# 0xastro/Cognitive-Radio-Network

Hardware: AMD Instinct MI355X
Metric: Msamples/s IQ through FFT+energy-detect, 4096-pt x 3ch; % HBM roofline (higher is better)
Workload: dtype f32

## Files before the change

### cognitive-radio-network_amd/csrc/crn_api.cpp

```cpp
#include <algorithm>
#include <cmath>
#include <cstdio>
#include <cstring>
#include <string>
#include <vector>

#include "crn_forms.h"
#include "crn_handle.h"
#include "crn_segments.h"

namespace crn {
static thread_local std::string g_err;
int fail(int code, const std::string &msg) {
  g_err = msg;
  return code;
}
}

void crn::handle_geometry(crn_handle *h, int *fft_len, int *device) {
  std::lock_guard<std::mutex> lk(h->tables_mu);
  *fft_len = h->cfg.fft_len;
  *device = h->device;
}

// ... 122 lines not shown
    h->tail_groups_per_wg = variant - 300;
    return CRN_OK;
  }
  if (variant >= 400 && variant <= 402) {
    h->deal_max_epochs = variant == 400 ? -1 : variant == 401 ? 0 : (int64_t)0x7fffffff;
    return CRN_OK;
  }
  if (variant < 0 || variant > crn::sense_num_variants()) return crn::fail(CRN_ERR_ARG, "variant out of range");
  if (!crn::sense_variant_available(variant))
    return crn::fail(CRN_ERR_ARG, "variant " + std::to_string(variant) + " is not a form of this library: the measurement variants (7, 17, 19-22, 26, 27) "
                                  "are compiled into libcrnsense_ab.so (make -C csrc ab), not into the shipped library; any other number names "
                                  "a form that no longer exists");
  h->variant = variant;
  return CRN_OK;
}

static void fill_plan_facts(const crn_handle *h, bool spectrum, crn::SenseParams &p) {
  p.hann_sym = h->cfg.window == CRN_WINDOW_HANN;
  p.aligned_shift = spectrum ? 0 : h->aligned_shift;
  p.acc_mask = h->variant == 2 ? 0xFFFFu : h->acc_mask;
  p.n_row_entries = h->n_row_entries;
  p.n_row_entries_shift = h->n_row_entries_shift;
  p.acc_mask_shift = h->variant == 2 ? 0xFFFFu : h->acc_mask_shift;
  p.cfar_on = h->cfar_on ? 1 : 0;
}

int crn_sense_kernel_info(crn_handle *h, char *name, int32_t name_len, int32_t *threads_per_block,
                          int32_t *lds_bytes, int32_t *epochs_per_block) {
  if (!h) return crn::fail(CRN_ERR_ARG, "null handle");
  std::lock_guard<std::mutex> lk(h->tables_mu);
  crn::SenseParams p{};
  p.L = h->cfg.fft_len;
  fill_plan_facts(h, false, p);
  const std::optional<crn::FormKey> k = crn::select_form(
      crn::make_form_query(p, h->cfg.fft_len, h->cfg.mode == CRN_MODE_REF_MAG, h->cfg.window != CRN_WINDOW_RECT, h->variant, false));
  if (!k) return crn::fail(CRN_ERR_STATE, "no kernel form for this handle");
  const crn::FormGeometry g = crn::form_geometry(*k);
  if (threads_per_block) *threads_per_block = g.threads;
  if (lds_bytes) *lds_bytes = g.lds_bytes;
  if (epochs_per_block) *epochs_per_block = g.epochs_per_block;
  if (name && name_len > 0) crn::form_name(*k, name, (size_t)name_len);
  return CRN_OK;
}

static int resolve_strides(const crn_handle *h, int32_t L, int64_t *epoch_stride, int *frame_stride) {
  const crn_cfg &c = h->cfg;
// ... 400 lines not shown
```

### cognitive-radio-network_amd/csrc/crn_butterflies.h

```cpp
#ifndef CRN_BUTTERFLIES_H
#define CRN_BUTTERFLIES_H
#include <hip/hip_runtime.h>
#include <type_traits>
#include <stdint.h>

#include "crn_forms.h"

namespace crn {

typedef float cx __attribute__((ext_vector_type(2)));
#define CRN_DEV static __device__ __forceinline__
#define CRN_HD static __host__ __device__ __forceinline__

#define CRN_C1 0.92387953251128674f
#define CRN_S1 0.38268343236508977f
#define CRN_H_ 0.70710678118654752f

#define CRN_PK_ADD "v_pk_add_f32 %0, %1, %2"
#define CRN_PK_SUB "v_pk_add_f32 %0, %1, %2 neg_lo:[0,1] neg_hi:[0,1]"
#define CRN_PK_ADD_MJ "v_pk_add_f32 %0, %1, %2 op_sel:[0,1] op_sel_hi:[1,0] neg_hi:[0,1]"
#define CRN_PK_SUB_MJ "v_pk_add_f32 %0, %1, %2 op_sel:[0,1] op_sel_hi:[1,0] neg_lo:[0,1]"
#define CRN_PK_MUL_T "v_pk_mul_f32 %0, %1, %2 op_sel_hi:[1,0]"
#define CRN_PK_MUL_D "v_pk_fma_f32 %0, %1, %2, %3 op_sel:[1,1,0] op_sel_hi:[0,1,1] neg_lo:[1,0,0]"
#define CRN_PK_MULCONJ_D "v_pk_fma_f32 %0, %1, %2, %3 op_sel:[1,1,0] op_sel_hi:[0,1,1] neg_hi:[1,0,0]"
// ... 157 lines not shown
CRN_HD void dft16_hann(const cx (&in)[16], cx (&out)[16], const cx (&wp)[4], const Hook &hook = Hook()) {
  using m = M<PK>;
  cx y[16];
#pragma unroll
  for (int i = 0; i < 16; i++) y[i] = in[i];
  static_for<4>([&](auto rc) {
    constexpr int r0 = decltype(rc)::value;
    constexpr int S = r0 & 1;
    const cx x0 = y[r0], x1 = y[r0 + 4], x2 = y[r0 + 8], x3 = y[r0 + 12];
    const cx w0 = wp[r0 / 2], w1 = wp[(r0 + 4) / 2];
    const cx s02 = m::template fma_w<S, false>(w0, m::sub(x0, x2), x2);
    const cx d02 = m::template fma_w<S, true>(w0, m::add(x0, x2), x2);
    const cx s13 = m::template fma_w<S, false>(w1, m::sub(x1, x3), x3);
    const cx d13 = m::template fma_w<S, true>(w1, m::add(x1, x3), x3);
    y[r0] = m::add(s02, s13);
    y[r0 + 8] = m::sub(s02, s13);
    y[r0 + 4] = m::add_mj(d02, d13);
    y[r0 + 12] = m::sub_mj(d02, d13);
    hook(r0);
  });
  dft16_level_b<PK>(y, out, hook);
}

template <bool PK, unsigned MASK>
CRN_HD void dft16_pruned(const cx (&in)[16], cx (&out)[16]) {
  using m = M<PK>;
  cx y[16];
#pragma unroll
  for (int i = 0; i < 16; i++) y[i] = in[i];
#pragma unroll
  for (int r0 = 0; r0 < 4; r0++) dft4<PK>(y[r0], y[r0 + 4], y[r0 + 8], y[r0 + 12]);
  const cx w1 = {CRN_C1, -CRN_S1}, w3 = {CRN_S1, -CRN_C1}, w9 = {-CRN_C1, CRN_S1};
  static_for<4>([&](auto ac) {
    constexpr int a0 = decltype(ac)::value;
    constexpr bool n0 = (MASK >> (a0 + 0)) & 1, n1 = (MASK >> (a0 + 4)) & 1, n2 = (MASK >> (a0 + 8)) & 1, n3 = (MASK >> (a0 + 12)) & 1;
    constexpr bool S = n0 || n2, D = n1 || n3;
    const cx b0 = y[4 * a0];
    if constexpr (a0 == 2) {
      const cx p = m::add_mj(y[9], y[9]), q = m::sub_mj(y[11], y[11]);
      if constexpr (S) {
        const cx s02 = m::add_mj(b0, y[10]), u = m::sub(p, q);
        if constexpr (n0) out[a0 + 0] = m::fma_h(u, s02);
        if constexpr (n2) out[a0 + 8] = m::fms_h(u, s02);
      }
      if constexpr (D) {
        const cx d02 = m::sub_mj(b0, y[10]), v = m::add(p, q);
        if constexpr (n1) out[a0 + 4] = m::fma_h_mj(v, d02);
        if constexpr (n3) out[a0 + 12] = m::fms_h_mj(v, d02);
      }
    } else {
      cx b1 = y[4 * a0 + 1], b3 = y[4 * a0 + 3];
      if constexpr (a0 == 1) { b1 = m::mul_c(b1, w1); b3 = m::mul_c(b3, w3); }
      if constexpr (a0 == 3) { b1 = m::mul_c(b1, w3); b3 = m::mul_c(b3, w9); }
      const cx r = a0 == 1 ? m::add_mj(y[4 * a0 + 2], y[4 * a0 + 2]) : a0 == 3 ? m::sub_mj(y[4 * a0 + 2], y[4 * a0 + 2]) : y[4 * a0 + 2];
      if constexpr (S) {
        const cx s02 = a0 == 0 ? m::add(b0, r) : a0 == 1 ? m::fma_h(r, b0) : m::fms_h(r, b0);
        const cx s13 = m::add(b1, b3);
        if constexpr (n0) out[a0 + 0] = m::add(s02, s13);
        if constexpr (n2) out[a0 + 8] = m::sub(s02, s13);
      }
      if constexpr (D) {
        const cx d02 = a0 == 0 ? m::sub(b0, r) : a0 == 1 ? m::fms_h(r, b0) : m::fma_h(r, b0);
        const cx d13 = m::sub(b1, b3);
        if constexpr (n1) out[a0 + 4] = m::add_mj(d02, d13);
        if constexpr (n3) out[a0 + 12] = m::sub_mj(d02, d13);
      }
    }
  });
}

template <bool PK, unsigned MSK, bool B2MJ = false>
CRN_HD void dft4_pruned(cx &a0, cx &a1, cx &a2, cx &a3) {
  using m = M<PK>;
  constexpr bool S = (MSK & 5u) != 0, D = (MSK & 10u) != 0;
  cx s02 = a0, d02 = a0, s13 = a1, d13 = a1;
  if constexpr (S) { s02 = B2MJ ? m::add_mj(a0, a2) : m::add(a0, a2); s13 = m::add(a1, a3); }
  if constexpr (D) { d02 = B2MJ ? m::sub_mj(a0, a2) : m::sub(a0, a2); d13 = m::sub(a1, a3); }
  if constexpr ((MSK & 1u) != 0) a0 = m::add(s02, s13);
  if constexpr ((MSK & 4u) != 0) a2 = m::sub(s02, s13);
  if constexpr ((MSK & 2u) != 0) a1 = m::add_mj(d02, d13);
  if constexpr ((MSK & 8u) != 0) a3 = m::sub_mj(d02, d13);
}

template <bool PK, unsigned M8>
CRN_HD void dft8_pruned(const cx (&in)[8], cx (&out)[8]) {
  using m = M<PK>;
  cx y[8];
#pragma unroll
  for (int i = 0; i < 8; i++) y[i] = in[i];
  constexpr unsigned need = (M8 | (M8 >> 4)) & 15u;
  dft4_pruned<PK, need>(y[0], y[2], y[4], y[6]);
  dft4_pruned<PK, need>(y[1], y[3], y[5], y[7]);
  if constexpr ((M8 & 0x01u) != 0) out[0] = m::add(y[0], y[1]);
  if constexpr ((M8 & 0x10u) != 0) out[4] = m::sub(y[0], y[1]);
  if constexpr ((M8 & 0x22u) != 0) {
    const cx p = m::add_mj(y[3], y[3]);
    if constexpr ((M8 & 0x02u) != 0) out[1] = m::fma_h(p, y[2]);
    if constexpr ((M8 & 0x20u) != 0) out[5] = m::fms_h(p, y[2]);
  }
  if constexpr ((M8 & 0x04u) != 0) out[2] = m::add_mj(y[4], y[5]);
  if constexpr ((M8 & 0x40u) != 0) out[6] = m::sub_mj(y[4], y[5]);
  if constexpr ((M8 & 0x88u) != 0) {
    const cx q = m::sub_mj(y[7], y[7]);
    if constexpr ((M8 & 0x08u) != 0) out[3] = m::fms_h(q, y[6]);
    if constexpr ((M8 & 0x80u) != 0) out[7] = m::fma_h(q, y[6]);
  }
// ... 24 lines not shown
```

### cognitive-radio-network_amd/csrc/crn_epoch_close.h

```cpp
#ifndef CRN_EPOCH_CLOSE_H
#define CRN_EPOCH_CLOSE_H
#include "crn_frame.h"

#ifdef CRN_AB_VARIANTS
#include "crn_frame_ab.h"
#else
namespace crn {
template <class C>
struct CloseTrace {
  CRN_DEV void workgroup_start(const SenseParams &, int) {}
  CRN_DEV void enter(const SenseParams &, long long, bool, int, int) {}
  CRN_DEV void stamp1() {}
  CRN_DEV void stamp2() {}
  CRN_DEV void stamp3() {}
  CRN_DEV void leave(const SenseParams &, long long, bool, int) {}
};
}
#endif

namespace crn {

template <int R3>
struct CloseImage {
  static constexpr int kFeat = spec_phys(Geo<R3>::N);
// ... 189 lines not shown
    constexpr auto next_live = [](int d) {
      for (int x = d + 1; x < R3; x++)
        for (int j = 0; j < J; j++)
          if ((acc_mask<C>() >> (j * R3 + x)) & 1u) return x;
      return (int)R3;
    };
    constexpr int kFirst = next_live(-1);
    float fsum = 0.f;
    constexpr bool SHIFTED = BinMap<C>::S != 0;
    constexpr int kEnt0 = SHIFTED ? 0 : kTabRowEntries;
    const int *ent_tab = SHIFTED ? p.row_entries_shift : p.band_tab;
    typename SWords<CAP>::T ent_next = s_load_row<CAP, (kEnt0 + kFirst * CAP) * 4>(ent_tab);
    static_for<R3>([&](auto dc) {
      constexpr int d = decltype(dc)::value;
      if constexpr (row_live(d)) {
        typename SWords<CAP>::T ent = ent_next;
        s_wait_row(ent);
        constexpr int dn = next_live(d);
        if constexpr (dn < R3) ent_next = s_load_row<CAP, (kEnt0 + dn * CAP) * 4>(ent_tab);
#pragma unroll
        for (int e = 0; e < CAP; e++) {
          const int w = ent[e];
          if (w != 0) {
            const int band = w >> 18, lo = (w >> 9) & 511, span = (w & 511) - lo;
            float v = 0.f;
#pragma unroll
            for (int j = 0; j < J; j++) {
              if (((AM >> (j * R3 + d)) & 1u) == 0) continue;
              const int base = BinMap<C>::q(a, m_lo, j);
              v += (unsigned)(base - lo) < (unsigned)span ? acc[j * R3 + d] : 0.f;
            }
            v = team_sum<TEAM>(v, tid);
            fsum += lane == band ? v : 0.f;
          }
        }
      }
    });
#pragma unroll
    for (int i = 0; i < 16; i++) acc[i] = 0.f;
    trace.stamp1();
    if constexpr (TPG > 1) {
      if (lane < 16) part[(tid / TEAM) * 16 + lane] = fsum;
      __syncthreads();
      trace.stamp2();
      if (t < TEAM && lane < 16) {
        thr_lane = thr[lane];
        fsum = 0.f;
#pragma unroll
        for (int w = 0; w < TPG; w++) fsum += part[(grp * TPG + w) * 16 + lane];
      }
    }
    trace.stamp3();
// ... 344 lines not shown
```

### cognitive-radio-network_amd/csrc/crn_forms.h

```cpp
#ifndef CRN_FORMS_H
#define CRN_FORMS_H
#include <optional>

#include "crn_kernels.h"

namespace crn {

enum : int {
  kSpread = 4,
  kLdsBlk = 32,
  kTw1C = 64,
  kRows = 256,
  kMulti = 512,
  kPrioValu = 1024,
#ifdef CRN_AB_VARIANTS
  kTrace = 4096,
#endif
  kRegBands = 8192,
  kHannSym = 16384,
  kTw2Early = 32768,
  kAlignedBands = 65536,
  kSc16 = 131072,
  kDeal = 1048576,
  kCfar = 2097152,
};

static constexpr unsigned kRefPlanRows = 0x8267u;

constexpr unsigned ref_acc_mask_shifted(int R3, int S) {
  const int seg[5][2] = {{0, 16}, {496, 511}, {55, 85}, {189, 222}, {300, 310}};
  const int J = 16 / R3, Sc = R3 / 2, N = 256 * R3;
  unsigned mask = 0;
  for (int s = 0; s < 5; s++)
    for (int k = seg[s][0] * Sc; k < seg[s][1] * Sc; k++) {
      const int ks = (k + S) & (N - 1);
      mask |= 1u << ((((ks & 255) >> 4) % J) * R3 + (ks >> 8));
    }
  return mask;
}
constexpr unsigned ref_acc_mask(int R3) { return ref_acc_mask_shifted(R3, 0); }
static_assert(ref_acc_mask(16) == kRefPlanRows, "N = 4096: register = 256-bin row");
static_assert(ref_acc_mask(2) == 0x85e1u && ref_acc_mask(4) == 0xbf73u && ref_acc_mask(8) == 0x9f9bu, "7, 12 and 11 registers at 512, 1024 and 2048 points");
static_assert(ref_acc_mask_shifted(16, kTw1cRowShift) == kRefPlanRows, "N = 4096: the plan reaches the same seven rows when they start 7 bins early");

constexpr int kCloseLdsBytes = kBandTabWords * 4 + 8 * 16 * 4;

struct LdsLayout {
  int group_bytes;
  int tw2;
  int tab;
  int part;
  int bytes;
  int slots;
  int round_values;
  constexpr size_t bytes_with_slots(int rounds, bool mag) const { return (size_t)bytes + (slots != 0 ? (size_t)rounds * round_values * (mag ? 4 : 8) : 0); }
};
constexpr LdsLayout lds_layout(int r3, int nbuf, bool dealt) {
  const int t = 16 * r3, groups = 256 / t, cplx = 8;
  LdsLayout l{};
  l.group_bytes = nbuf * 16 * (t + r3) * cplx;
  l.tw2 = groups * l.group_bytes;
  l.tab = l.tw2 + 16 * r3 * cplx;
  l.part = l.tab + kBandTabWords * 4;
  l.bytes = l.tab + kCloseLdsBytes;
  l.slots = dealt ? l.bytes : 0;
  l.round_values = groups * 256 * r3;
// ... 154 lines not shown
```

### cognitive-radio-network_amd/csrc/crn_frame.h

```cpp
#ifndef CRN_FRAME_H
#define CRN_FRAME_H
#include "crn_butterflies.h"
#include "crn_forms.h"

namespace crn {
template <int R3>
struct Geo {
  static constexpr int N = 256 * R3;
  static constexpr int T = 16 * R3;
  static constexpr int GROUPS = 256 / T;
  static constexpr int ROW = T + R3;
  static constexpr int GROUP_CPLX = 16 * ROW;
  static constexpr int J = 16 / R3;
  static constexpr bool XWAVE = (T > 64);
  static constexpr int TEAM = T < 64 ? T : 64;
};

__host__ __device__ constexpr int spec_phys(int k) { return k + (k >> 4); }

typedef unsigned int v2u __attribute__((ext_vector_type(2)));

template <bool NT, bool SC = false>
CRN_DEV cx ld_iq(__amdgpu_buffer_rsrc_t rsrc, unsigned voff, unsigned soff) {
  if constexpr (SC) {
// ... 40 lines not shown
CRN_DEV void mask_frame(cx (&u)[16], int t, int L) {
  constexpr int T = Geo<R3>::T;
#pragma unroll
  for (int r = 0; r < 16; r++)
    if (t + T * r >= L) u[r] = cx{0.f, 0.f};
}

CRN_DEV void wave_sync() {
  __builtin_amdgcn_fence(__ATOMIC_RELEASE, "wavefront");
  __builtin_amdgcn_wave_barrier();
}

template <int R3_, int NBUF_, bool PREFETCH_, bool NT_, bool MAG_, bool WIN_, bool TW2LDS_, int OCC_, bool FULL_, bool PK_, int OPT_ = 0>
struct Cfg {
  static constexpr int OPT = OPT_;
  static constexpr int R3 = R3_, NBUF = NBUF_, OCC = OCC_;
  static constexpr bool PREFETCH = PREFETCH_, NT = NT_, MAG = MAG_, WIN = WIN_, TW2LDS = TW2LDS_, FULL = FULL_,
                        PK = PK_;
  static constexpr bool SC16 = (OPT_ & kSc16) != 0;
  static constexpr unsigned SB = SC16 ? 4u : 8u;
};

template <class C>
struct BinMap {
  static constexpr int S = (C::OPT & kTw1C) != 0 ? kTw1cRowShift : 0;
  static_assert(S == 0 || C::R3 == 16, "the compressed pass-1 table exists at N = 4096");
  CRN_DEV constexpr int q(int a, int m_lo, int j) { return lane_coord<S>(a, m_lo, j, Geo<C::R3>::J); }
  CRN_DEV constexpr int bin(int a, int m_lo, int j, int d) { return bin_of<S>(q(a, m_lo, j), d, Geo<C::R3>::N); }
};
template <class C>
struct FrameCtx {
  cx tw1[16];
  cx tw2[16];
  float win[16];
  cx winp[4];
  float acc[16];
  const cx *tw2_lds;
  int wave;
  int grp_epoch_stride;
  unsigned lds_base;
  cx *gbuf;
  int t, a, m_lo, L;
  unsigned park_off;
  float Kf, invK;
};

template <int R3, bool NT, bool SC = false>
struct SpreadLoads {
  cx (&nx)[16];
  __amdgpu_buffer_rsrc_t rsrc;
  unsigned voff, soff;
  int pass;
  bool half;
  int L;
  __device__ __forceinline__ void operator()(int k) const {
    if (pass > 1 || (half && pass != 0)) return;
    const int idx = pass * 8 + k;
    __builtin_amdgcn_sched_barrier(0);
    nx[idx] = ld_iq<NT, SC>(rsrc, voff, Geo<R3>::T * idx < L ? soff + (unsigned)(Geo<R3>::T * idx * (SC ? 4 : 8)) : kOffNowhere);
    __builtin_amdgcn_sched_barrier(0);
  }
// ... 6 lines not shown
  using m = M<C::PK>;
  if constexpr (C::SC16) unpack_frame(u);
  if constexpr (!C::FULL) mask_frame<C::R3>(u, c.t, c.L);
  if constexpr (C::WIN && (C::OPT & kHannSym) != 0) {
    dft16_hann<C::PK>(u, v, c.winp, hook);
  } else {
    if constexpr (C::WIN) {
#pragma unroll
      for (int r = 0; r < 16; r++) u[r] = cx{u[r].x * c.win[r], u[r].y * c.win[r]};
    }
    dft16<C::PK>(u, v, hook);
  }
  if constexpr ((C::OPT & kTw1C) != 0) {
#pragma unroll
    for (int i = 1; i <= 8; i++) v[i] = m::mul(v[i], c.tw1[i]);
#pragma unroll
    for (int i = 9; i < 16; i++) v[i] = m::mul_conj(v[i], c.tw1[16 - i]);
  } else {
#pragma unroll
    for (int i = 1; i < 16; i++) v[i] = m::mul(v[i], c.tw1[i]);
  }
}
template <class C>
CRN_DEV void ph_x1_write(const cx (&v)[16], cx *buf, FrameCtx<C> &c) {
#pragma unroll
  for (int i = 0; i < 16; i++) buf[i * Geo<C::R3>::ROW + c.t] = v[i];
}
#define CRN_RD(i) "ds_read_b64 %" #i ", %16 offset:%" 
template <int STRIDE_BYTES>
CRN_DEV void lds_read16_b64(cx (&u)[16], const cx *base) {
  const unsigned addr = (unsigned)(size_t)base;
  asm volatile(
      "ds_read_b64 %0, %16 offset:%17\n\tds_read_b64 %1, %16 offset:%18\n\tds_read_b64 %2, %16 offset:%19\n\t"
      "ds_read_b64 %3, %16 offset:%20\n\tds_read_b64 %4, %16 offset:%21\n\tds_read_b64 %5, %16 offset:%22\n\t"
      "ds_read_b64 %6, %16 offset:%23\n\tds_read_b64 %7, %16 offset:%24\n\tds_read_b64 %8, %16 offset:%25\n\t"
      "ds_read_b64 %9, %16 offset:%26\n\tds_read_b64 %10, %16 offset:%27\n\tds_read_b64 %11, %16 offset:%28\n\t"
      "ds_read_b64 %12, %16 offset:%29\n\tds_read_b64 %13, %16 offset:%30\n\tds_read_b64 %14, %16 offset:%31\n\t"
      "ds_read_b64 %15, %16 offset:%32\n\ts_waitcnt lgkmcnt(0)"
      : "=&v"(u[0]), "=&v"(u[1]), "=&v"(u[2]), "=&v"(u[3]), "=&v"(u[4]), "=&v"(u[5]), "=&v"(u[6]), "=&v"(u[7]), "=&v"(u[8]),
        "=&v"(u[9]), "=&v"(u[10]), "=&v"(u[11]), "=&v"(u[12]), "=&v"(u[13]), "=&v"(u[14]), "=&v"(u[15])
      : "v"(addr), "n"(0 * STRIDE_BYTES), "n"(1 * STRIDE_BYTES), "n"(2 * STRIDE_BYTES), "n"(3 * STRIDE_BYTES),
        "n"(4 * STRIDE_BYTES), "n"(5 * STRIDE_BYTES), "n"(6 * STRIDE_BYTES), "n"(7 * STRIDE_BYTES),
        "n"(8 * STRIDE_BYTES), "n"(9 * STRIDE_BYTES), "n"(10 * STRIDE_BYTES), "n"(11 * STRIDE_BYTES),
        "n"(12 * STRIDE_BYTES), "n"(13 * STRIDE_BYTES), "n"(14 * STRIDE_BYTES), "n"(15 * STRIDE_BYTES)
      : "memory");
}
#undef CRN_RD

template <int STRIDE_BYTES>
// ... 8 lines not shown
        "n"(4 * STRIDE_BYTES), "n"(5 * STRIDE_BYTES), "n"(6 * STRIDE_BYTES), "n"(7 * STRIDE_BYTES)
      : "memory");
}

template <int STRIDE_BYTES>
CRN_DEV void lds_issue8_b64(cx (&w)[8], const cx *base) {
  const unsigned addr = (unsigned)(size_t)base;
  asm volatile(
      "ds_read_b64 %0, %8 offset:%9\n\tds_read_b64 %1, %8 offset:%10\n\tds_read_b64 %2, %8 offset:%11\n\t"
      "ds_read_b64 %3, %8 offset:%12\n\tds_read_b64 %4, %8 offset:%13\n\tds_read_b64 %5, %8 offset:%14\n\t"
      "ds_read_b64 %6, %8 offset:%15\n\tds_read_b64 %7, %8 offset:%16"
      : "=&v"(w[0]), "=&v"(w[1]), "=&v"(w[2]), "=&v"(w[3]), "=&v"(w[4]), "=&v"(w[5]), "=&v"(w[6]), "=&v"(w[7])
      : "v"(addr), "n"(0 * STRIDE_BYTES), "n"(1 * STRIDE_BYTES), "n"(2 * STRIDE_BYTES), "n"(3 * STRIDE_BYTES),
        "n"(4 * STRIDE_BYTES), "n"(5 * STRIDE_BYTES), "n"(6 * STRIDE_BYTES), "n"(7 * STRIDE_BYTES)
      : "memory");
}
CRN_DEV void lds_wait8(cx (&w)[8]) {
  asm volatile("s_waitcnt lgkmcnt(0)"
               : "+v"(w[0]), "+v"(w[1]), "+v"(w[2]), "+v"(w[3]), "+v"(w[4]), "+v"(w[5]), "+v"(w[6]), "+v"(w[7])
               :
               : "memory");
}

template <class C>
CRN_DEV void ph_x1_read(cx (&u)[16], cx *buf, FrameCtx<C> &c) {
  const cx *row = buf + c.a * Geo<C::R3>::ROW;
  if constexpr ((C::OPT & kLdsBlk) != 0) {
    lds_read16_b64<C::R3 * 8>(u, row + c.m_lo);
    return;
  }
#pragma unroll
  for (int i = 0; i < 16; i++) u[i] = row[C::R3 * i + c.m_lo];
}
template <class C, class Hook = NoHook>
CRN_DEV void ph_pass2(cx (&u)[16], cx (&v)[16], FrameCtx<C> &c, const Hook &hook = Hook()) {
  using m = M<C::PK>;
  if constexpr (C::TW2LDS && (C::OPT & kLdsBlk) != 0 && (C::OPT & kTw2Early) != 0) {
    cx wa[8], wb[8];
    lds_issue8_b64<C::R3 * 8>(wa, c.tw2_lds + 1 * C::R3 + c.m_lo);
    dft16<C::PK>(u, v, hook);
    lds_wait8(wa);
    lds_issue8_b64<C::R3 * 8>(wb, c.tw2_lds + 8 * C::R3 + c.m_lo);
#pragma unroll
    for (int i = 1; i <= 8; i++) v[i] = m::mul(v[i], wa[i - 1]);
    lds_wait8(wb);
#pragma unroll
    for (int i = 9; i < 16; i++) v[i] = m::mul(v[i], wb[i - 8]);
    return;
  }
// ... 10 lines not shown
  }
#pragma unroll
  for (int i = 1; i < 16; i++) v[i] = m::mul(v[i], C::TW2LDS ? c.tw2_lds[i * C::R3 + c.m_lo] : c.tw2[i]);
}
template <class C>
CRN_DEV void ph_x2_write(const cx (&v)[16], cx *buf, FrameCtx<C> &c) {
  constexpr int R3 = C::R3, J = Geo<R3>::J;
  cx *row = buf + c.a * Geo<R3>::ROW;
#pragma unroll
  for (int cc = 0; cc < 16; cc++) row[cc * R3 + c.m_lo + cc / J] = v[cc];
}
template <class C>
CRN_DEV void ph_x2_read(cx (&u)[16], cx *buf, FrameCtx<C> &c) {
  constexpr int R3 = C::R3, J = Geo<R3>::J;
  const cx *row = buf + c.a * Geo<R3>::ROW;
  if constexpr ((C::OPT & kLdsBlk) != 0 && R3 == 16) {
    lds_read16_b64<8>(u, row + 17 * c.m_lo);
    return;
  }
#pragma unroll
  for (int j = 0; j < J; j++)
#pragma unroll
    for (int mm = 0; mm < R3; mm++) u[j * R3 + mm] = row[(c.m_lo * J + j) * R3 + mm + c.m_lo];
}
template <class C>
CRN_DEV void ph_pass3(cx (&u)[16], cx (&v)[16]) {
  constexpr int R3 = C::R3, J = Geo<R3>::J;
  using m = M<C::PK>;
  if constexpr (R3 == 16) {
    dft16<C::PK>(u, v);
  } else if constexpr (R3 == 8) {
#pragma unroll
    for (int j = 0; j < J; j++) {
      cx in8[8], out8[8];
#pragma unroll
      for (int mm = 0; mm < 8; mm++) in8[mm] = u[j * 8 + mm];
      dft8<C::PK>(in8, out8);
#pragma unroll
      for (int mm = 0; mm < 8; mm++) v[j * 8 + mm] = out8[mm];
    }
  } else if constexpr (R3 == 4) {
#pragma unroll
    for (int j = 0; j < J; j++) {
      dft4<C::PK>(u[j * 4], u[j * 4 + 1], u[j * 4 + 2], u[j * 4 + 3]);
#pragma unroll
      for (int mm = 0; mm < 4; mm++) v[j * 4 + mm] = u[j * 4 + mm];
// ... 74 lines not shown
#pragma unroll
    for (int i = 0; i < 16; i++) slot[i * T + c.t] = v[i];
  }
}
template <class C>
CRN_DEV void replay_parked(FrameCtx<C> &c, unsigned park_base, int K) {
  constexpr int T = Geo<C::R3>::T;
  constexpr unsigned kSlotBytes = (unsigned)Geo<C::R3>::N * (C::MAG ? 4u : 8u);
  for (int f = 0; f < K; f++) {
    const unsigned off = park_base + (unsigned)f * kSlotBytes;
#pragma unroll
    for (int i = 0; i < 16; i++) {
      if constexpr (C::MAG) {
        const float mag = reinterpret_cast<const lds_park_f32 *>(off)[i * T + c.t];
        c.acc[i] = fmaf(mag, c.invK, c.acc[i]);
      } else {
        const cx x = reinterpret_cast<const lds_park_cx *>(off)[i * T + c.t];
        c.acc[i] = fmaf(x.y, x.y, fmaf(x.x, x.x, c.acc[i]));
      }
    }
  }
}

template <class C>
CRN_DEV void ph_pass3_acc(cx (&u)[16], FrameCtx<C> &c) {
  if constexpr ((C::OPT & kDeal) != 0) {
    ph_pass3_park<C>(u, c);
    return;
  }
  cx v[16];
  constexpr unsigned MASK = acc_mask<C>();
  if constexpr (MASK == 0xFFFFu) {
    ph_pass3<C>(u, v);
  } else {
#pragma unroll
    for (int i = 0; i < 16; i++) v[i] = cx{0.f, 0.f};
    ph_pass3_pruned<C, MASK>(u, v);
  }
#pragma unroll
  for (int i = 0; i < 16; i++) {
    if (((MASK >> i) & 1u) == 0) continue;
    if constexpr (C::MAG) {
      const float mag = __builtin_amdgcn_sqrtf(fmaf(v[i].x, v[i].x, v[i].y * v[i].y));
      c.acc[i] = fmaf(mag, c.invK, c.acc[i]);
    } else {
      c.acc[i] = fmaf(v[i].y, v[i].y, fmaf(v[i].x, v[i].x, c.acc[i]));
    }
  }
}

template <class C>
CRN_DEV void group_sync() {
  if constexpr (Geo<C::R3>::XWAVE) __syncthreads();
  else wave_sync();
}

template <class C, bool HALF = false>
CRN_DEV void frame_compute(cx (&u)[16], FrameCtx<C> &c, int f, cx (&nx)[16], __amdgpu_buffer_rsrc_t rsrc, unsigned voff, unsigned soff_next) {
  using G = Geo<C::R3>;
  static_assert((C::OPT & kSpread) != 0, "the kernels fetch the next frame from inside the current one's butterflies");
  cx *buf = c.gbuf + (C::NBUF == 2 ? (f & 1) * G::GROUP_CPLX : 0);
  cx v[16];
  const int Lrows = C::FULL ? G::N : c.L;
  const SpreadLoads<C::R3, C::NT, C::SC16> h1{nx, rsrc, voff, soff_next, 0, HALF, Lrows}, h2{nx, rsrc, voff, soff_next, 1, HALF, Lrows};
  constexpr bool PV = (C::OPT & kPrioValu) != 0;
  if constexpr (PV) __builtin_amdgcn_s_setprio(1);
  ph_pass1<C>(u, v, c, h1);
  if constexpr (PV) __builtin_amdgcn_s_setprio(0);
  if constexpr (G::XWAVE && C::NBUF == 1) __syncthreads();
  ph_x1_write<C>(v, buf, c);
  group_sync<C>();
  ph_x1_read<C>(u, buf, c);
  if constexpr (PV) __builtin_amdgcn_s_setprio(1);
  ph_pass2<C>(u, v, c, h2);
  if constexpr (PV) __builtin_amdgcn_s_setprio(0);
  wave_sync();
  ph_x2_write<C>(v, buf, c);
  wave_sync();
  ph_x2_read<C>(u, buf, c);
  ph_pass3_acc<C>(u, c);
}

}
#endif
```

### cognitive-radio-network_amd/csrc/crn_handle.h

```cpp
#ifndef CRN_HANDLE_H
#define CRN_HANDLE_H
#include <hip/hip_runtime.h>

#include <atomic>
#include <mutex>

#include "crn_internal.h"

struct crn_handle {
  explicit crn_handle(int dev) : device(dev) {}
  const int device;
  crn_cfg cfg;
  int variant = 0;
  int groups_per_wg = 0;
  int64_t tail_groups = -1;
  int tail_groups_per_wg = 0;
  std::atomic<int64_t> n_dealt{0};
  int64_t deal_max_epochs = -1;
  int n_row_entries = 0;
  int aligned_shift = 0;
  std::atomic<int> n_rings{0};
  int n_cus = 256;
  size_t lds_budget = 64 * 1024;
  unsigned acc_mask = 0xFFFFu;
  int n_row_entries_shift = 0;
  unsigned acc_mask_shift = 0xFFFFu;
  bool cfar_on = false;
  crn_cfar_params_ex cfar{};
  void *d_tables = nullptr;
  const float2 *d_tw1 = nullptr, *d_tw2 = nullptr;
  const float *d_window = nullptr, *d_thresh = nullptr;
  const int *d_band_seg_begin = nullptr, *d_seg_lo = nullptr, *d_seg_hi = nullptr;
  const int *d_band_bins_begin = nullptr, *d_band_bins = nullptr, *d_band_tab = nullptr, *d_band_c2 = nullptr, *d_row_entries_shift = nullptr;
  const double *d_wih = nullptr, *d_who = nullptr;
  void *d_scratch = nullptr;
  size_t scratch_bytes = 0;
  double window_power = 0.0;
  double wire_full_scale = 32768.0;
  float *d_nf_scratch = nullptr;
  void *h_small = nullptr;
  size_t h_small_bytes = 0;
  void *h_results = nullptr;
  size_t h_results_bytes = 0;
  std::mutex tables_mu;
  std::mutex nf_mu;
  struct UpdateSlot {
    float thresh[CRN_MAX_BANDS];
    double w_ih[CRN_ANN_IN + 1][CRN_ANN_HID + 1];
    double w_ho[CRN_ANN_HID + 1][CRN_ANN_OUT + 1];
// ... 24 lines not shown
```

### cognitive-radio-network_amd/csrc/crn_kernels.h

```cpp
#ifndef CRN_KERNELS_H
#define CRN_KERNELS_H

#include <hip/hip_runtime.h>
#include <stdint.h>

namespace crn {

constexpr int kBandTabWords = 656;
constexpr int kRowEntryWords = 32;
constexpr int kTabSegBegin = 0, kTabSegBeginWords = 96;
constexpr int kTabSegLo = 96, kTabSegHi = 256, kTabSegWords = 160;
constexpr int kTabThresh = 416, kTabThreshWords = 80;
constexpr int kTabRowEntries = 512;
constexpr int kTabWih = 544, kTabWihWords = 60, kTabWho = 604, kTabWhoWords = 48;
static_assert(kTabSegBegin + kTabSegBeginWords <= kTabSegLo && kTabSegLo + kTabSegWords <= kTabSegHi && kTabSegHi + kTabSegWords <= kTabThresh &&
              kTabThresh + kTabThreshWords <= kTabRowEntries && kTabRowEntries + kRowEntryWords <= kTabWih && kTabWih % 2 == 0 &&
              kTabWih + kTabWihWords <= kTabWho && kTabWho + kTabWhoWords <= kBandTabWords, "band_tab: regions in order, disjoint, inside the table");

constexpr int kTw1cRowShift = 7;
template <int S>
constexpr int lane_coord(int a, int g, int j, int J) {
  if constexpr (S == 0) return a + 16 * (g * J + j);
  else return ((a + S) & 15) + 16 * (g * J + j);
}
template <int S>
constexpr int bin_of(int q, int d, int N) {
  if constexpr (S == 0) return q + 256 * d;
  else return (q + 256 * d - S) & (N - 1);
}

enum { CRN_DECIDE_ANN_K = 0, CRN_DECIDE_THRESHOLD_K = 1, CRN_DECIDE_NONE_K = 2 };
enum { CRN_CFAR_CA_K = 0, CRN_CFAR_GO_K = 1, CRN_CFAR_SO_K = 2, CRN_CFAR_OS_K = 3 };

struct SenseParams {
  const float2 *iq;
  long long n_epochs;
  long long epoch_stride;
  long long total_samples;
  int frame_stride;
  int L;
  int K;
  int groups_per_wg;
  long long n_big_wgs;
  int tail_groups_per_wg;
  const float2 *tw1;
  const float2 *tw2;
  const float *window;
  const int *band_tab;
  const int *band_seg_begin;
  const int *seg_lo;
  const int *seg_hi;
  const float *thresh;
// ... 6 lines not shown
  int n_row_entries;
  int aligned_shift;
  int hann_sym;
  unsigned acc_mask;
  int deal_rounds;
  float wire_unscale;
  float *features;
  double *ann_out;
  int32_t *decision;
  uint8_t *occupancy;
  float *spectrum;
  int cfar_on;
  int cfar_guard;
  int cfar_train;
  int cfar_min_bins;
  float cfar_scale;
  uint32_t *cfar_mask;
  int32_t *cfar_band_bins;
  int cfar_method;
  int cfar_rank;
  const int *row_entries_shift;
  int n_row_entries_shift;
  unsigned acc_mask_shift;
};

struct SynthParams {
  float2 *iq;
  long long n_epochs;
  long long samples_per_epoch;
  unsigned long long seed;
  float noise_sigma;
  float tone_amp;
  int tones;
  int fft_len;
  int n_active;
  int active_band0;
  const int *band_bins_begin;
  const int *band_bins;
  const int *band_c2;
  int32_t *truth;
  int pu_model;
  int signal_kind;
  float signal_rms;
  long long epochs_per_stream;
  float adc_scale;
};
// ... 36 lines not shown
```

### cognitive-radio-network_amd/csrc/crn_sense_kernel.h

```cpp
#ifndef CRN_SENSE_KERNEL_H
#define CRN_SENSE_KERNEL_H
#include <atomic>
#include <utility>

#include "crn_epoch_close.h"

namespace crn {
template <int R3, int SB = 8>
CRN_DEV __amdgpu_buffer_rsrc_t group_rsrc(const SenseParams &p, long long eg, int span = 1) {
  using G = Geo<R3>;
  const long long first = eg * G::GROUPS * p.epoch_stride;
  long long left = (p.total_samples - first) * SB;
  const long long window = ((long long)span * G::GROUPS * p.epoch_stride + (long long)p.K * p.frame_stride + G::N) * SB;
  if (left > window) left = window;
  if (left < 0) left = 0;
  char *base = reinterpret_cast<char *>(const_cast<float2 *>(p.iq)) + first * SB;
  return __builtin_amdgcn_make_buffer_rsrc(base, 0, (int)left, 0x00020000);
}

struct StreamSpan {
  long long g0;
  int epw, n_local;
};
template <int R3>
// ... 20 lines not shown
  constexpr bool NT = C::NT, SC = C::SC16;
  constexpr unsigned SB = C::SB;
  using G = Geo<R3>;
  constexpr int T = G::T;
  constexpr LdsLayout kLds = lds_layout(R3, NBUF, false);
  extern __shared__ __attribute__((aligned(16))) cx lds[];

  const int tid = threadIdx.x;
  const int grp = tid / T;
  const int t = tid % T;
  const int a = t / R3;
  const int m_lo = t % R3;

  FrameCtx<C> c;
  c.t = t;
  c.a = a;
  c.m_lo = m_lo;
  c.L = p.L;
  c.gbuf = lds + grp * (kLds.group_bytes / (int)sizeof(cx));
  c.wave = __builtin_amdgcn_readfirstlane(tid >> 6);
  c.grp_epoch_stride = 1;
  c.lds_base = (unsigned)__builtin_amdgcn_readfirstlane((int)lds_offset(lds));
  c.tw2_lds = lds_at<cx>(lds, kLds.tw2);
  CloseTrace<C>::workgroup_start(p, tid);
  const int K = p.K;
  c.Kf = (float)K;
  c.invK = 1.0f / (float)K;

  constexpr unsigned kNowhere = 0x80000000u;
  const unsigned voff = (unsigned)(grp * (unsigned)p.epoch_stride + t) * SB;
  const unsigned fbytes = (unsigned)p.frame_stride * SB;
  cx ua[16], ub[16];
  static_assert((C::OPT & kMulti) != 0 && C::PREFETCH, "the kernels are streaming workgroups with the prefetch spread through the butterflies");
  constexpr bool kEarlyLoad = !C::WIN;
  if constexpr (kEarlyLoad) {
    const StreamSpan sp0 = stream_span<R3>(p);
    load_frame<R3, NT, SC>(ua, group_rsrc<R3, (int)SB>(p, sp0.g0, sp0.epw), voff, 0u, C::FULL ? G::N : c.L);
  }

#pragma unroll
  for (int i = 1; i < ((C::OPT & kTw1C) != 0 ? 9 : 16); i++) c.tw1[i] = reinterpret_cast<const cx *>(p.tw1)[i * T + t];
  if constexpr (!C::TW2LDS) {
#pragma unroll
    for (int i = 1; i < 16; i++) c.tw2[i] = reinterpret_cast<const cx *>(p.tw2)[i * R3 + m_lo];
  }
  if constexpr (C::WIN && (C::OPT & kHannSym) != 0) {
// ... 302 lines not shown
```

### cognitive-radio-network_amd/csrc/crn_tables.cpp

```cpp
#include <algorithm>
#include <cmath>
#include <cstring>
#include <string>
#include <vector>

#include "crn_handle.h"
#include "crn_kernels.h"

static_assert(crn::kTabSegBeginWords >= CRN_MAX_BANDS + 1 && crn::kTabSegWords >= CRN_MAX_SEGS && crn::kTabThreshWords >= CRN_MAX_BANDS,
              "band_tab: the band plan's regions hold the largest plan");
static_assert(crn::kTabWihWords * sizeof(int) == sizeof(crn_cfg::ann_w_ih) && sizeof(crn_cfg::ann_w_ih) == 30 * sizeof(double) &&
              crn::kTabWhoWords * sizeof(int) == sizeof(crn_cfg::ann_w_ho) && sizeof(crn_cfg::ann_w_ho) == 24 * sizeof(double),
              "band_tab: the weight regions hold 30 and 24 doubles");

static float2 twiddle(long long q, int n) {
  q %= n;
  const double ang = -2.0 * M_PI * (double)q / (double)n;
  return make_float2((float)std::cos(ang), (float)std::sin(ang));
}

int crn::validate(const crn_cfg *c) {
  if (!c) return crn::fail(CRN_ERR_ARG, "null cfg");
  if (c->abi_version != CRN_ABI_VERSION) return crn::fail(CRN_ERR_ARG, "cfg.abi_version mismatch");
  if (const int n = c->fft_len; n != 512 && n != 1024 && n != 2048 && n != 4096) return crn::fail(CRN_ERR_ARG, "fft_len must be 512, 1024, 2048 or 4096");
// ... 79 lines not shown
    struct RowPiece { int d, band, lo, hi; };
    std::vector<RowPiece> pieces;
    for (int b = 0; b < cfg.n_bands; b++)
      for (int sg = seg_begin[b]; sg < seg_begin[b + 1]; sg++)
        for (int d = seg_lo[sg] >> 8; seg_lo[sg] < seg_hi[sg] && d <= (seg_hi[sg] - 1) >> 8; d++) {
          const int lo = std::max(seg_lo[sg], 256 * d) - 256 * d, hi = std::min(seg_hi[sg], 256 * (d + 1)) - 256 * d;
          pieces.push_back({d, b, lo, hi});
        }
    const int cap = crn::kRowEntryWords / R3;
    bool fits = cfg.n_bands <= 16 && !pieces.empty();
    std::vector<int> used(16, 0);
    for (const RowPiece &pc : pieces)
      if (++used[pc.d] > cap) fits = false;
    if (fits) {
      std::fill(used.begin(), used.end(), 0);
      for (const RowPiece &pc : pieces) band_tab[crn::kTabRowEntries + pc.d * cap + used[pc.d]++] = (pc.band << 18) | (pc.lo << 9) | pc.hi;
      n_row_entries = (int)pieces.size();
    }
  }

  std::vector<int> row_entries_shift(crn::kRowEntryWords, 0);
  int n_row_entries_shift = 0;
  unsigned acc_mask_shift = 0;
  {
    const int S = crn::kTw1cRowShift, J = 16 / R3, cap = crn::kRowEntryWords / R3;
    struct RowPiece { int d, band, lo, hi; };
    std::vector<RowPiece> pieces;
    auto cut = [&](int band, int lo, int hi) {
      for (int d = lo >> 8; lo < hi && d <= (hi - 1) >> 8; d++)
        pieces.push_back({d, band, std::max(lo, 256 * d) - 256 * d, std::min(hi, 256 * (d + 1)) - 256 * d});
    };
    for (int b = 0; b < cfg.n_bands; b++)
      for (int sg = seg_begin[b]; sg < seg_begin[b + 1]; sg++) {
        const int lo = seg_lo[sg] + S, hi = seg_hi[sg] + S;
        cut(b, std::min(lo, N), std::min(hi, N));
        cut(b, std::max(lo, N) - N, std::max(hi, N) - N);
        for (int k = seg_lo[sg]; k < seg_hi[sg]; k++) {
          const int ks = (k + S) & (N - 1);
          acc_mask_shift |= 1u << ((((ks & 255) >> 4) % J) * R3 + (ks >> 8));
        }
      }
    bool fits = cfg.n_bands <= 16 && !pieces.empty();
    std::vector<int> used(16, 0);
    for (const RowPiece &pc : pieces)
      if (++used[pc.d] > cap) fits = false;
    if (fits) {
      std::fill(used.begin(), used.end(), 0);
      for (const RowPiece &pc : pieces) row_entries_shift[pc.d * cap + used[pc.d]++] = (pc.band << 18) | (pc.lo << 9) | pc.hi;
      n_row_entries_shift = (int)pieces.size();
    }
  }

  std::vector<int> band_c2(std::max(cfg.n_bands, 1), 0);
  for (int b = 0; b < cfg.n_bands; b++) {
    int lo = N, hi = -N;
    for (int i = bins_begin[b]; i < bins_begin[b + 1]; i++) {
      const int k = bins[i] >= N / 2 ? bins[i] - N : bins[i];
      lo = std::min(lo, k);
      hi = std::max(hi, k);
    }
    band_c2[b] = bins_begin[b + 1] > bins_begin[b] ? lo + hi : 0;
  }
// ... 18 lines not shown
  size_t total = 0;
  for (auto &p : parts) {
    p.off = total;
    total = align_up(total + p.bytes, 256);
  }
  std::vector<char> host(total, 0);
  for (auto &p : parts) std::memcpy(host.data() + p.off, p.src, p.bytes);
  void *slab = nullptr;
  hipError_t e = hipMalloc(&slab, total);
  if (e != hipSuccess) return crn::fail(CRN_ERR_NOMEM, std::string("hipMalloc(tables): ") + hipGetErrorString(e));
  e = hipMemcpy(slab, host.data(), total, hipMemcpyHostToDevice);
  if (e != hipSuccess) {
    (void)hipFree(slab);
    return crn::fail(CRN_ERR_DEVICE, std::string("hipMemcpy(tables): ") + hipGetErrorString(e));
  }
  if (h->d_tables) (void)hipFree(h->d_tables);
  h->cfg = cfg;
  h->window_power = window_power;
  h->aligned_shift = aligned_shift;
  h->n_row_entries = n_row_entries;
  h->acc_mask = acc_mask;
  h->n_row_entries_shift = n_row_entries_shift;
  h->acc_mask_shift = acc_mask_shift;
  h->d_tables = slab;
  char *base = static_cast<char *>(h->d_tables);
  h->d_tw1 = reinterpret_cast<const float2 *>(base + parts[0].off);
  h->d_tw2 = reinterpret_cast<const float2 *>(base + parts[1].off);
  h->d_window = reinterpret_cast<const float *>(base + parts[2].off);
  h->d_thresh = reinterpret_cast<const float *>(base + parts[3].off);
  h->d_band_seg_begin = reinterpret_cast<const int *>(base + parts[4].off);
  h->d_seg_lo = reinterpret_cast<const int *>(base + parts[5].off);
  h->d_seg_hi = reinterpret_cast<const int *>(base + parts[6].off);
  h->d_band_bins_begin = reinterpret_cast<const int *>(base + parts[7].off);
  h->d_band_bins = reinterpret_cast<const int *>(base + parts[8].off);
  h->d_wih = reinterpret_cast<const double *>(base + parts[9].off);
  h->d_who = reinterpret_cast<const double *>(base + parts[10].off);
  h->d_band_tab = reinterpret_cast<const int *>(base + parts[11].off);
  h->d_band_c2 = reinterpret_cast<const int *>(base + parts[12].off);
  h->d_row_entries_shift = reinterpret_cast<const int *>(base + parts[13].off);
  return CRN_OK;
}
```

Before: 822,600.

## Share pass-2 transpose across the workgroup and prune pass-3 rows per wave

Replaces the per-wave pass-2/pass-3 LDS exchange with a workgroup-wide transpose that uses a skewed row layout and 128-bit LDS reads. Each wave then handles one quarter of the columns and runs a pass-3 DFT pruned to only the rows that hold bins the band plan uses. The pruned rows are compile-time masks built from a hardcoded reference band layout; a runtime cell-mask check from the tables falls back to the general path otherwise. The change trades wave-local syncs for __syncthreads and adds a specialization that only pays off for that band plan. The pruned dft4 is also applied to the first radix-4 stage of dft16_pruned.

Measured after the change: 830,500, median of 6. About the same (+1.0%).

```diff
diff --git a/cognitive-radio-network_amd/csrc/crn_api.cpp b/cognitive-radio-network_amd/csrc/crn_api.cpp
--- a/cognitive-radio-network_amd/csrc/crn_api.cpp
+++ b/cognitive-radio-network_amd/csrc/crn_api.cpp
@@ -168,6 +168,7 @@
   p.n_row_entries = h->n_row_entries;
   p.n_row_entries_shift = h->n_row_entries_shift;
   p.acc_mask_shift = h->variant == 2 ? 0xFFFFu : h->acc_mask_shift;
+  p.cell_mask_shift = h->cell_mask_shift;
   p.cfar_on = h->cfar_on ? 1 : 0;
 }
 
diff --git a/cognitive-radio-network_amd/csrc/crn_butterflies.h b/cognitive-radio-network_amd/csrc/crn_butterflies.h
--- a/cognitive-radio-network_amd/csrc/crn_butterflies.h
+++ b/cognitive-radio-network_amd/csrc/crn_butterflies.h
@@ -203,14 +203,33 @@
   dft16_level_b<PK>(y, out, hook);
 }
 
+template <bool PK, unsigned MSK, bool B2MJ = false>
+CRN_HD void dft4_pruned(cx &a0, cx &a1, cx &a2, cx &a3) {
+  using m = M<PK>;
+  constexpr bool S = (MSK & 5u) != 0, D = (MSK & 10u) != 0;
+  cx s02 = a0, d02 = a0, s13 = a1, d13 = a1;
+  if constexpr (S) { s02 = B2MJ ? m::add_mj(a0, a2) : m::add(a0, a2); s13 = m::add(a1, a3); }
+  if constexpr (D) { d02 = B2MJ ? m::sub_mj(a0, a2) : m::sub(a0, a2); d13 = m::sub(a1, a3); }
+  if constexpr ((MSK & 1u) != 0) a0 = m::add(s02, s13);
+  if constexpr ((MSK & 4u) != 0) a2 = m::sub(s02, s13);
+  if constexpr ((MSK & 2u) != 0) a1 = m::add_mj(d02, d13);
+  if constexpr ((MSK & 8u) != 0) a3 = m::sub_mj(d02, d13);
+}
+
 template <bool PK, unsigned MASK>
 CRN_HD void dft16_pruned(const cx (&in)[16], cx (&out)[16]) {
   using m = M<PK>;
   cx y[16];
 #pragma unroll
   for (int i = 0; i < 16; i++) y[i] = in[i];
-#pragma unroll
-  for (int r0 = 0; r0 < 4; r0++) dft4<PK>(y[r0], y[r0 + 4], y[r0 + 8], y[r0 + 12]);
+  constexpr unsigned NEED = (MASK | (MASK >> 4) | (MASK >> 8) | (MASK >> 12)) & 15u;
+  if constexpr (NEED == 15u) {
+#pragma unroll
+    for (int r0 = 0; r0 < 4; r0++) dft4<PK>(y[r0], y[r0 + 4], y[r0 + 8], y[r0 + 12]);
+  } else {
+#pragma unroll
+    for (int r0 = 0; r0 < 4; r0++) dft4_pruned<PK, NEED>(y[r0], y[r0 + 4], y[r0 + 8], y[r0 + 12]);
+  }
   const cx w1 = {CRN_C1, -CRN_S1}, w3 = {CRN_S1, -CRN_C1}, w9 = {-CRN_C1, CRN_S1};
   static_for<4>([&](auto ac) {
     constexpr int a0 = decltype(ac)::value;
@@ -250,19 +269,6 @@
   });
 }
 
-template <bool PK, unsigned MSK, bool B2MJ = false>
-CRN_HD void dft4_pruned(cx &a0, cx &a1, cx &a2, cx &a3) {
-  using m = M<PK>;
-  constexpr bool S = (MSK & 5u) != 0, D = (MSK & 10u) != 0;
-  cx s02 = a0, d02 = a0, s13 = a1, d13 = a1;
-  if constexpr (S) { s02 = B2MJ ? m::add_mj(a0, a2) : m::add(a0, a2); s13 = m::add(a1, a3); }
-  if constexpr (D) { d02 = B2MJ ? m::sub_mj(a0, a2) : m::sub(a0, a2); d13 = m::sub(a1, a3); }
-  if constexpr ((MSK & 1u) != 0) a0 = m::add(s02, s13);
-  if constexpr ((MSK & 4u) != 0) a2 = m::sub(s02, s13);
-  if constexpr ((MSK & 2u) != 0) a1 = m::add_mj(d02, d13);
-  if constexpr ((MSK & 8u) != 0) a3 = m::sub_mj(d02, d13);
-}
-
 template <bool PK, unsigned M8>
 CRN_HD void dft8_pruned(const cx (&in)[8], cx (&out)[8]) {
   using m = M<PK>;
diff --git a/cognitive-radio-network_amd/csrc/crn_epoch_close.h b/cognitive-radio-network_amd/csrc/crn_epoch_close.h
--- a/cognitive-radio-network_amd/csrc/crn_epoch_close.h
+++ b/cognitive-radio-network_amd/csrc/crn_epoch_close.h
@@ -235,12 +235,16 @@
         for (int e = 0; e < CAP; e++) {
           const int w = ent[e];
           if (w != 0) {
+            if constexpr (kX2Wg<C>) {
+              if ((w & 511) <= 64 * c.wave || ((w >> 9) & 511) >= 64 * c.wave + 64) continue;
+            }
             const int band = w >> 18, lo = (w >> 9) & 511, span = (w & 511) - lo;
             float v = 0.f;
 #pragma unroll
             for (int j = 0; j < J; j++) {
               if (((AM >> (j * R3 + d)) & 1u) == 0) continue;
-              const int base = BinMap<C>::q(a, m_lo, j);
+              int base = BinMap<C>::q(a, m_lo, j);
+              if constexpr (kX2Wg<C>) base = BinMap<C>::q(BinMap<C>::a_of(t), BinMap<C>::g_of(t), j);
               v += (unsigned)(base - lo) < (unsigned)span ? acc[j * R3 + d] : 0.f;
             }
             v = team_sum<TEAM>(v, tid);
diff --git a/cognitive-radio-network_amd/csrc/crn_forms.h b/cognitive-radio-network_amd/csrc/crn_forms.h
--- a/cognitive-radio-network_amd/csrc/crn_forms.h
+++ b/cognitive-radio-network_amd/csrc/crn_forms.h
@@ -42,6 +42,22 @@
 static_assert(ref_acc_mask(16) == kRefPlanRows, "N = 4096: register = 256-bin row");
 static_assert(ref_acc_mask(2) == 0x85e1u && ref_acc_mask(4) == 0xbf73u && ref_acc_mask(8) == 0x9f9bu, "7, 12 and 11 registers at 512, 1024 and 2048 points");
 static_assert(ref_acc_mask_shifted(16, kTw1cRowShift) == kRefPlanRows, "N = 4096: the plan reaches the same seven rows when they start 7 bins early");
+
+constexpr unsigned long long ref_cells_shifted(int S) {
+  const int seg[5][2] = {{0, 16}, {496, 511}, {55, 85}, {189, 222}, {300, 310}};
+  unsigned long long cells = 0;
+  for (int s = 0; s < 5; s++)
+    for (int k = seg[s][0] * 8; k < seg[s][1] * 8; k++) cells |= x2wg_cell((k + S) & 4095);
+  return cells;
+}
+inline constexpr unsigned long long kRefCells = ref_cells_shifted(kTw1cRowShift);
+constexpr unsigned ref_quarter_rows(int w) { return (unsigned)(kRefCells >> (16 * w)) & 0xFFFFu; }
+static_assert(ref_quarter_rows(0) == 0x0045u && ref_quarter_rows(1) == 0x0245u && ref_quarter_rows(2) == 0x8247u && ref_quarter_rows(3) == 0x8062u,
+              "quarter 0: rows {0, 2, 6}; 1: {0, 2, 6, 9}; 2: {0, 1, 2, 6, 9, 15}; 3: {1, 5, 6, 15}");
+static_assert((ref_quarter_rows(0) | ref_quarter_rows(1) | ref_quarter_rows(2) | ref_quarter_rows(3)) == kRefPlanRows, "the cells lie in the seven rows and reach each of them");
+constexpr bool ref_cells_hold(unsigned long long cells) { return (cells & ~kRefCells) == 0; }
+
+constexpr int x2wg_row_skew(int a) { return 2 * (a >> 1); }
 
 constexpr int kCloseLdsBytes = kBandTabWords * 4 + 8 * 16 * 4;
 
diff --git a/cognitive-radio-network_amd/csrc/crn_frame.h b/cognitive-radio-network_amd/csrc/crn_frame.h
--- a/cognitive-radio-network_amd/csrc/crn_frame.h
+++ b/cognitive-radio-network_amd/csrc/crn_frame.h
@@ -86,9 +86,14 @@
 };
 
 template <class C>
+inline constexpr bool kX2Wg = C::R3 == 16 && (C::OPT & kTw1C) != 0 && (C::OPT & kRegBands) != 0 && C::NBUF == 1;
+
+template <class C>
 struct BinMap {
   static constexpr int S = (C::OPT & kTw1C) != 0 ? kTw1cRowShift : 0;
   static_assert(S == 0 || C::R3 == 16, "the compressed pass-1 table exists at N = 4096");
+  CRN_DEV constexpr int a_of(int t) { return kX2Wg<C> ? x2wg_a(t) : t / C::R3; }
+  CRN_DEV constexpr int g_of(int t) { return kX2Wg<C> ? x2wg_g(t) : t % C::R3; }
   CRN_DEV constexpr int q(int a, int m_lo, int j) { return lane_coord<S>(a, m_lo, j, Geo<C::R3>::J); }
   CRN_DEV constexpr int bin(int a, int m_lo, int j, int d) { return bin_of<S>(q(a, m_lo, j), d, Geo<C::R3>::N); }
 };
@@ -101,6 +106,7 @@
   float acc[16];
   const cx *tw2_lds;
   int wave;
+  bool quarters;
   int grp_epoch_stride;
   unsigned lds_base;
   cx *gbuf;
@@ -153,9 +159,14 @@
   }
 }
 template <class C>
+CRN_DEV constexpr int x_row(int a) {
+  if constexpr (kX2Wg<C>) return a * Geo<C::R3>::ROW + x2wg_row_skew(a);
+  else return a * Geo<C::R3>::ROW;
+}
+template <class C>
 CRN_DEV void ph_x1_write(const cx (&v)[16], cx *buf, FrameCtx<C> &c) {
 #pragma unroll
-  for (int i = 0; i < 16; i++) buf[i * Geo<C::R3>::ROW + c.t] = v[i];
+  for (int i = 0; i < 16; i++) buf[x_row<C>(i) + c.t] = v[i];
 }
 #define CRN_RD(i) "ds_read_b64 %" #i ", %16 offset:%" 
 template <int STRIDE_BYTES>
@@ -210,9 +221,28 @@
                : "memory");
 }
 
+typedef float v4f __attribute__((ext_vector_type(4)));
+CRN_DEV void lds_read8_b128(cx (&u)[16], const cx *base) {
+  const unsigned addr = (unsigned)(size_t)base;
+  v4f q0, q1, q2, q3, q4, q5, q6, q7;
+  asm volatile(
+      "ds_read_b128 %0, %8\n\tds_read_b128 %1, %8 offset:16\n\tds_read_b128 %2, %8 offset:32\n\tds_read_b128 %3, %8 offset:48\n\t"
+      "ds_read_b128 %4, %8 offset:64\n\tds_read_b128 %5, %8 offset:80\n\tds_read_b128 %6, %8 offset:96\n\tds_read_b128 %7, %8 offset:112"
+      : "=&v"(q0), "=&v"(q1), "=&v"(q2), "=&v"(q3), "=&v"(q4), "=&v"(q5), "=&v"(q6), "=&v"(q7)
+      : "v"(addr)
+      : "memory");
+  asm volatile("s_waitcnt lgkmcnt(0)" : "+v"(q0), "+v"(q1), "+v"(q2), "+v"(q3), "+v"(q4), "+v"(q5), "+v"(q6), "+v"(q7) : : "memory");
+  const v4f q[8] = {q0, q1, q2, q3, q4, q5, q6, q7};
+#pragma unroll
+  for (int i = 0; i < 8; i++) {
+    u[2 * i] = cx{q[i].x, q[i].y};
+    u[2 * i + 1] = cx{q[i].z, q[i].w};
+  }
+}
+
 template <class C>
 CRN_DEV void ph_x1_read(cx (&u)[16], cx *buf, FrameCtx<C> &c) {
-  const cx *row = buf + c.a * Geo<C::R3>::ROW;
+  const cx *row = buf + x_row<C>(c.a);
   if constexpr ((C::OPT & kLdsBlk) != 0) {
     lds_read16_b64<C::R3 * 8>(u, row + c.m_lo);
     return;
@@ -269,6 +299,16 @@
   for (int j = 0; j < J; j++)
 #pragma unroll
     for (int mm = 0; mm < R3; mm++) u[j * R3 + mm] = row[(c.m_lo * J + j) * R3 + mm + c.m_lo];
+}
+template <class C>
+CRN_DEV void ph_x2wg_write(const cx (&v)[16], cx *buf, FrameCtx<C> &c) {
+  cx *slot = buf + x_row<C>(c.a) + c.m_lo;
+#pragma unroll
+  for (int cc = 0; cc < 16; cc++) slot[16 * cc] = v[cc];
+}
+template <class C>
+CRN_DEV void ph_x2wg_read(cx (&u)[16], cx *buf, FrameCtx<C> &c) {
+  lds_read8_b128(u, buf + x_row<C>(x2wg_a(c.t)) + 16 * x2wg_g(c.t));
 }
 template <class C>
 CRN_DEV void ph_pass3(cx (&u)[16], cx (&v)[16]) {
@@ -389,14 +429,9 @@
   }
 }
 
-template <class C>
-CRN_DEV void ph_pass3_acc(cx (&u)[16], FrameCtx<C> &c) {
-  if constexpr ((C::OPT & kDeal) != 0) {
-    ph_pass3_park<C>(u, c);
-    return;
-  }
+template <class C, unsigned MASK>
+CRN_DEV void pass3_acc_rows(cx (&u)[16], FrameCtx<C> &c) {
   cx v[16];
-  constexpr unsigned MASK = acc_mask<C>();
   if constexpr (MASK == 0xFFFFu) {
     ph_pass3<C>(u, v);
   } else {
@@ -414,6 +449,39 @@
       c.acc[i] = fmaf(v[i].y, v[i].y, fmaf(v[i].x, v[i].x, c.acc[i]));
     }
   }
+}
+
+template <class C, unsigned MASK>
+CRN_DEV void pass3_acc_quarter(cx (&u)[16], FrameCtx<C> &c) {
+  static_assert(C::R3 == 16 && !C::MAG, "the plain 4096-point kernel: energy mode");
+  cx v[16];
+  ph_x2wg_read<C>(u, c.gbuf, c);
+  ph_pass3_pruned<C, MASK>(u, v);
+  static_for<16>([&](auto ic) {
+    constexpr int i = decltype(ic)::value;
+    if constexpr (((MASK >> i) & 1u) != 0) c.acc[i] = fmaf(v[i].y, v[i].y, fmaf(v[i].x, v[i].x, c.acc[i]));
+  });
+}
+
+template <class C>
+CRN_DEV void ph_pass3_acc(cx (&u)[16], FrameCtx<C> &c) {
+  if constexpr ((C::OPT & kDeal) != 0) {
+    ph_pass3_park<C>(u, c);
+    return;
+  }
+  if constexpr (kX2Wg<C> && (C::OPT & kRows) != 0) {
+    if (c.quarters) {
+      switch (c.wave) {
+        case 0: pass3_acc_quarter<C, ref_quarter_rows(0)>(u, c); break;
+        case 1: pass3_acc_quarter<C, ref_quarter_rows(1)>(u, c); break;
+        case 2: pass3_acc_quarter<C, ref_quarter_rows(2)>(u, c); break;
+        default: pass3_acc_quarter<C, ref_quarter_rows(3)>(u, c); break;
+      }
+      return;
+    }
+  }
+  if constexpr (kX2Wg<C>) ph_x2wg_read<C>(u, c.gbuf, c);
+  pass3_acc_rows<C, acc_mask<C>()>(u, c);
 }
 
 template <class C>
@@ -441,10 +509,15 @@
   if constexpr (PV) __builtin_amdgcn_s_setprio(1);
   ph_pass2<C>(u, v, c, h2);
   if constexpr (PV) __builtin_amdgcn_s_setprio(0);
-  wave_sync();
-  ph_x2_write<C>(v, buf, c);
-  wave_sync();
-  ph_x2_read<C>(u, buf, c);
+  if constexpr (kX2Wg<C>) {
+    ph_x2wg_write<C>(v, buf, c);
+    __syncthreads();
+  } else {
+    wave_sync();
+    ph_x2_write<C>(v, buf, c);
+    wave_sync();
+    ph_x2_read<C>(u, buf, c);
+  }
   ph_pass3_acc<C>(u, c);
 }
 
diff --git a/cognitive-radio-network_amd/csrc/crn_handle.h b/cognitive-radio-network_amd/csrc/crn_handle.h
--- a/cognitive-radio-network_amd/csrc/crn_handle.h
+++ b/cognitive-radio-network_amd/csrc/crn_handle.h
@@ -25,6 +25,7 @@
   unsigned acc_mask = 0xFFFFu;
   int n_row_entries_shift = 0;
   unsigned acc_mask_shift = 0xFFFFu;
+  unsigned long long cell_mask_shift = ~0ull;
   bool cfar_on = false;
   crn_cfar_params_ex cfar{};
   void *d_tables = nullptr;
diff --git a/cognitive-radio-network_amd/csrc/crn_kernels.h b/cognitive-radio-network_amd/csrc/crn_kernels.h
--- a/cognitive-radio-network_amd/csrc/crn_kernels.h
+++ b/cognitive-radio-network_amd/csrc/crn_kernels.h
@@ -28,6 +28,10 @@
   if constexpr (S == 0) return q + 256 * d;
   else return (q + 256 * d - S) & (N - 1);
 }
+
+constexpr int x2wg_a(int t) { return t & 15; }
+constexpr int x2wg_g(int t) { return t >> 4; }
+constexpr unsigned long long x2wg_cell(int ks) { return 1ull << ((((ks & 255) >> 6) << 4) + (ks >> 8)); }
 
 enum { CRN_DECIDE_ANN_K = 0, CRN_DECIDE_THRESHOLD_K = 1, CRN_DECIDE_NONE_K = 2 };
 enum { CRN_CFAR_CA_K = 0, CRN_CFAR_GO_K = 1, CRN_CFAR_SO_K = 2, CRN_CFAR_OS_K = 3 };
@@ -80,6 +84,7 @@
   const int *row_entries_shift;
   int n_row_entries_shift;
   unsigned acc_mask_shift;
+  unsigned long long cell_mask_shift;
 };
 
 struct SynthParams {
diff --git a/cognitive-radio-network_amd/csrc/crn_sense_kernel.h b/cognitive-radio-network_amd/csrc/crn_sense_kernel.h
--- a/cognitive-radio-network_amd/csrc/crn_sense_kernel.h
+++ b/cognitive-radio-network_amd/csrc/crn_sense_kernel.h
@@ -66,6 +66,7 @@
   c.grp_epoch_stride = 1;
   c.lds_base = (unsigned)__builtin_amdgcn_readfirstlane((int)lds_offset(lds));
   c.tw2_lds = lds_at<cx>(lds, kLds.tw2);
+  if constexpr (kX2Wg<C> && (C::OPT & kRows) != 0) c.quarters = ref_cells_hold(p.cell_mask_shift);
   CloseTrace<C>::workgroup_start(p, tid);
   const int K = p.K;
   c.Kf = (float)K;
diff --git a/cognitive-radio-network_amd/csrc/crn_tables.cpp b/cognitive-radio-network_amd/csrc/crn_tables.cpp
--- a/cognitive-radio-network_amd/csrc/crn_tables.cpp
+++ b/cognitive-radio-network_amd/csrc/crn_tables.cpp
@@ -125,6 +125,7 @@
   std::vector<int> row_entries_shift(crn::kRowEntryWords, 0);
   int n_row_entries_shift = 0;
   unsigned acc_mask_shift = 0;
+  unsigned long long cell_mask_shift = 0;
   {
     const int S = crn::kTw1cRowShift, J = 16 / R3, cap = crn::kRowEntryWords / R3;
     struct RowPiece { int d, band, lo, hi; };
@@ -141,6 +142,7 @@
         for (int k = seg_lo[sg]; k < seg_hi[sg]; k++) {
           const int ks = (k + S) & (N - 1);
           acc_mask_shift |= 1u << ((((ks & 255) >> 4) % J) * R3 + (ks >> 8));
+          if (R3 == 16) cell_mask_shift |= crn::x2wg_cell(ks);
         }
       }
     bool fits = cfg.n_bands <= 16 && !pieces.empty();
@@ -205,6 +207,7 @@
   h->acc_mask = acc_mask;
   h->n_row_entries_shift = n_row_entries_shift;
   h->acc_mask_shift = acc_mask_shift;
+  h->cell_mask_shift = R3 == 16 ? cell_mask_shift : ~0ull;
   h->d_tables = slab;
   char *base = static_cast<char *>(h->d_tables);
   h->d_tw1 = reinterpret_cast<const float2 *>(base + parts[0].off);
```
